# GoekeLab/m6anet

Hardware: AMD Instinct MI355X
Metric: DRACH sites/sec at num_iterations=1000 (higher is better)
Workload: dtype f32

## Files before the change

m6anet_amd/csrc/m6a_api.hip:

```cpp
#include "m6a_ctx.h"

#if !defined(__HIP_DEVICE_COMPILE__)
#ifndef M6A_MT_JUMP_PATH
#error "build with -DM6A_MT_JUMP_PATH=\"<repo>/m6anet_amd/assets/mt19937_jump.bin\" (m6anet_amd/build.py does)"
#endif
asm(".section .rodata\n"
    ".global m6a_mt_jump_blob\n.global m6a_mt_jump_blob_end\n.hidden m6a_mt_jump_blob\n.hidden m6a_mt_jump_blob_end\n.balign 64\n"
    "m6a_mt_jump_blob:\n.incbin \"" M6A_MT_JUMP_PATH "\"\n"
    "m6a_mt_jump_blob_end:\n.byte 0\n.previous\n");
#endif

namespace {

thread_local std::string g_create_error;

std::mutex g_live_mu;
std::vector<m6a_ctx *> g_live;
void join_background_setups()
{
    std::lock_guard<std::mutex> g(g_live_mu);
    for (m6a_ctx *c : g_live)
        if (c->warm.joinable()) c->warm.join();
    g_live.clear();
}
// ... 553 lines not shown
    hipLaunchKernelGGL(bag_verify_kernel, dim3(1), dim3(256), 0, st, c->d_minmax, c->d_hist, (unsigned long long)c->bag_min,
                       (unsigned long long)c->bag_max, (unsigned long long)c->n_reads, hash, c->d_err);
    HIPCHK(c, hipGetLastError());
    c->side_work = true;
    return M6A_OK;
}

int launch_encode(m6a_ctx *c, const float *X, const uint8_t *km, const int64_t *off, int64_t S,
                  int64_t R, float *rp)
{
    if (R <= 0 || S <= 0) return M6A_OK;
    EncArgs a;
    a.X = X; a.site_kmers = km; a.off = off; a.wfrag = c->d_wfrag; a.emb = c->d_emb; a.read_prob = rp;
    a.wfrag2 = c->d_wfrag2; a.w1e_tab = c->d_w1e; a.bn = c->d_w1e + M6A_W1E_FLOATS; a.err = c->d_err;
    a.n_sites = S; a.n_reads = R; a.n_tiles = (R + 31) / 32; a.b3 = c->b3;
    a.clk = c->prof.clk_for(0);
#ifdef M6A_AB_W3
    const int64_t max_waves = (int64_t)c->n_cu * 12;
#else
    const int64_t max_waves = (int64_t)c->n_cu * 8;
#endif
    a.tiles_per_wave = (a.n_tiles + max_waves - 1) / max_waves;
    const int64_t waves = (a.n_tiles + a.tiles_per_wave - 1) / a.tiles_per_wave;
    const unsigned blocks = (unsigned)((waves + 3) / 4);
    const bool fits32 = S < 0x7ffffff0LL && a.n_tiles < 0x7ffffff0LL;
    if (c->enc_variant == 2 && !fits32) return fail(c, M6A_EUNSUPPORTED, "12-slot encoder: more than 2^31 sites or tiles");
    const bool scalar_chain = c->bag_min >= M6A_CSITE_MIN_BAG && fits32;
    const bool csite = c->enc_variant == 2 || (c->enc_variant == 4 && scalar_chain);
    const bool site16 = !csite && c->enc_variant != 3 && scalar_chain;
    c->enc_variant_used = csite ? "csite12" : "general16";
// ... 831 lines not shown
```

m6anet_amd/csrc/m6a_ctx.h:

```cpp
#pragma once
#include <hip/hip_runtime.h>
#include <dlfcn.h>
#include <sys/mman.h>

#include <algorithm>
#include <atomic>
#include <cmath>
#include <cstdarg>
#include <cstdio>
#include <cstdlib>
#include <cstring>
#include <condition_variable>
#include <functional>
#include <memory>
#include <mutex>
#include <new>
#include <string>
#include <thread>
#include <vector>

#include "m6a.h"
#include "m6a_kernels.h"
#include "m6a_host_cpus.h"

// ... 193 lines not shown
    int rt_presize = 0;
    uint32_t rt_credit_seed = 0; int64_t rt_credit_A = 0, rt_credit = 0;
    struct Job {
        bool open = false;
        int failed = 0;
        std::string failed_msg;
        int T = 0, K = 0; float thr = 0.f; uint32_t seed = 0; int64_t bs = 1, spb = 1;
        std::vector<int64_t> off;
        int64_t S = 0, R = 0;
        int n_sub = 0; size_t sub_bytes = 0, o_goff = 0, o_km = 0, o_x = 0;
        int64_t cap_sites = 0, cap_reads = 0;
        std::vector<char *> pin;
        std::vector<hipEvent_t> ev_h2d, ev_enc;
        std::vector<char> used;
        int64_t item = 0;
        int64_t fill_sites = 0, fill_reads = 0, fill_min = INT64_MAX;
        bool cur_ready = false;
        int64_t chunks = 0;
    } job;
    DevBuf gSite, gMod, gP;
    DevBuf jX, jP, jOff;
    DevBuf mt_scratch; int64_t mt_polys_G = 0;
    std::vector<int> iter_of;
    std::thread warm;
    void *comm = nullptr;
    int comm_rank = 0, comm_world = 0;
    Profiler prof;
    const char *pool_variant = "none";
};

namespace m6a_detail {
// ... 44 lines not shown
```

m6anet_amd/csrc/m6a_job.hip:

```cpp
#include "m6a_ctx.h"

using namespace m6a_detail;

namespace m6a_detail {

int grow_keep(m6a_ctx *c, DevBuf &b, size_t used_bytes, size_t need_bytes)
{
    if (need_bytes <= b.cap) return M6A_OK;
    const size_t want = std::max(need_bytes + need_bytes / 8 + 256, b.cap * 2);
    void *np_ = nullptr;
    HIPCHK(c, hipMalloc(&np_, want));
    if (b.p && used_bytes) {
        if (c->stg.s_h2d) HIPCHK(c, hipStreamSynchronize(c->stg.s_h2d));
        HIPCHK(c, hipMemcpyAsync(np_, b.p, used_bytes, hipMemcpyDeviceToDevice, c->stream));
        HIPCHK(c, hipStreamSynchronize(c->stream));
    }
    if (b.p) (void)hipFree(b.p);
    b.p = np_; b.cap = want;
    return M6A_OK;
}

int job_setup_ring(m6a_ctx *c)
{
    auto &j = c->job;
// ... 52 lines not shown
    const int64_t ns = j.fill_sites, nr = j.fill_reads, s0 = j.S - ns, r0 = j.R - nr;
    int rc = grow_keep(c, c->jP, (size_t)r0 * 4, (size_t)std::max<int64_t>(j.R, 1) * 4);
    if (rc) return rc;
    rc = grow_keep(c, c->jOff, (size_t)(s0 + 1) * 8, (size_t)(j.S + 1) * 8);
    if (rc) return rc;
    if (j.used[(size_t)sub]) HIPCHK(c, hipStreamWaitEvent(g.s_h2d, j.ev_enc[(size_t)sub], 0));
    HIPCHK(c, hipMemcpyAsync(dev, pin, (size_t)(ns + 1) * 8, hipMemcpyHostToDevice, g.s_h2d));
    HIPCHK(c, hipMemcpyAsync((int64_t *)c->jOff.p + s0, pin + j.o_goff, (size_t)(ns + 1) * 8, hipMemcpyHostToDevice, g.s_h2d));
    if (!dX) {
        HIPCHK(c, hipMemcpyAsync(dev + j.o_km, pin + j.o_km, (size_t)ns * 3, hipMemcpyHostToDevice, g.s_h2d));
        if (nr) HIPCHK(c, hipMemcpyAsync(dev + j.o_x, pin + j.o_x, (size_t)nr * M6A_N_FEATURES * 4, hipMemcpyHostToDevice, g.s_h2d));
    }
    HIPCHK(c, hipEventRecord(j.ev_h2d[(size_t)sub], g.s_h2d));
    HIPCHK(c, hipStreamWaitEvent(c->stream, j.ev_h2d[(size_t)sub], 0));
    if (nr) {
        c->bag_min = j.fill_min; c->n_reads = nr;
        rc = launch_encode(c, dX ? dX : (const float *)(dev + j.o_x), dK ? dK : (const uint8_t *)(dev + j.o_km), (const int64_t *)dev, ns, nr,
                           (float *)c->jP.p + r0);
        if (rc) return rc;
    }
    HIPCHK(c, hipEventRecord(j.ev_enc[(size_t)sub], c->stream));
    j.used[(size_t)sub] = 1;
    j.item++; j.chunks++;
    j.fill_sites = 0; j.fill_reads = 0; j.fill_min = INT64_MAX; j.cur_ready = false;
    return M6A_OK;
}

void job_append_offsets(m6a_ctx *c, char *pin, const int64_t *off, int64_t i, int64_t k)
{
    auto &j = c->job;
    int64_t *ol = (int64_t *)pin, *og = (int64_t *)(pin + j.o_goff);
    if (j.fill_sites == 0) { ol[0] = 0; og[0] = j.R; }
    const int64_t base = off[i], lbase = j.fill_reads, gbase = j.R;
    int64_t mn = j.fill_min;
    for (int64_t t = 0; t < k; t++) {
        const int64_t e = off[i + t + 1] - base, n = off[i + t + 1] - off[i + t];
        ol[j.fill_sites + t + 1] = lbase + e;
        og[j.fill_sites + t + 1] = gbase + e;
        j.off.push_back(gbase + e);
        mn = n < mn ? n : mn;
    }
    j.fill_min = mn;
    const int64_t nr = off[i + k] - base;
    j.fill_sites += k; j.fill_reads += nr; j.S += k; j.R += nr;
}

int job_feed_impl(m6a_ctx *c, const float *X, const uint8_t *km, const int64_t *off, int64_t n, bool dev)
{
    auto &j = c->job;
    if (off[0] != 0) return fail(c, M6A_EINVAL, "off[0] must be 0");
    for (int64_t s = 0; s < n; s++) if (off[s + 1] < off[s]) return fail(c, M6A_EINVAL, "off[] must be non-decreasing");
    int rc;
    if (dev) {
        rc = job_flush(c);
        if (rc) return rc;
        for (int64_t i = 0; i < n;) {
            char *pin;
// ... 55 lines not shown
        return fail(c, M6A_EINVAL, "job offset %lld does not start a flush group for batch_size=%lld save_per_batch=%lld",
                    (long long)c->job_offset, (long long)bs, (long long)spb);
    HIPCHK(c, hipSetDevice(c->device));
    rc = job_setup_ring(c);
    if (rc) return rc;
    auto &j = c->job;
    j.T = T; j.K = K; j.thr = thr; j.seed = seed; j.bs = bs; j.spb = spb;
    try {
        j.off.clear();
        j.off.reserve((size_t)std::max<int64_t>(expect_sites, 1 << 16) + 1);
        j.off.push_back(0);
    } catch (const std::bad_alloc &) {
        return fail(c, M6A_ENOMEM, "out of host memory");
    }
    j.S = j.R = 0; j.item = 0; j.chunks = 0; j.failed = 0; j.failed_msg.clear();
    j.fill_sites = j.fill_reads = 0; j.fill_min = INT64_MAX; j.cur_ready = false;
    std::fill(j.used.begin(), j.used.end(), 0);
    HIPCHK(c, hipStreamSynchronize(c->stg.s_h2d));
    if (expect_reads) { rc = grow_keep(c, c->jP, 0, (size_t)expect_reads * 4); if (rc) return rc; }
    if (expect_sites) { rc = grow_keep(c, c->jOff, 0, (size_t)(expect_sites + 1) * 8); if (rc) return rc; }
    j.open = true;
    return M6A_OK;
}

int m6a_job_feed(m6a_ctx *c, const float *X, const uint8_t *km, const int64_t *off, int64_t n_sites)
{
    settle(c);
    if (!c) return M6A_EINVAL;
    auto &j = c->job;
    if (!j.open) return fail(c, M6A_EINVAL, "no streaming job is open (m6a_job_begin)");
    if (j.failed) { c->err = j.failed_msg; return j.failed; }
// ... 123 lines not shown
```

m6anet_amd/csrc/m6a_kernels.h:

```cpp
#ifndef M6A_KERNELS_H
#define M6A_KERNELS_H
#include <hip/hip_runtime.h>
#include <stdint.h>

#define M6A_BAG_LDS 1024
#define M6A_WFRAG_FLOATS (136 * 64)
#define M6A_WFRAG2_FLOATS (25 * 64)
#define M6A_W1E_FLOATS (35 * 32)
#define M6A_BN_FLOATS (5 * 2 * 16 * 2)
#define M6A_MEAN_STACK 32
#define M6A_CSITE_MIN_BAG 16
#define M6A_TABLE_MAX_N 32
#define M6A_REG_STACK 8
#define M6A_RTAB_MAX_N 4096
#define M6A_RTAB_SMALL_N 1024
#define M6A_RTAB_U8_MAX_N 256
#define M6A_HIST_BINS (M6A_RTAB_MAX_N + 2)

__host__ __device__ inline unsigned long long m6a_bin_weight(int i)
{
    unsigned long long z = (unsigned long long)(i + 1) * 0x9E3779B97F4A7C15ull;
    z = (z ^ (z >> 30)) * 0xBF58476D1CE4E5B9ull;
    z = (z ^ (z >> 27)) * 0x94D049BB133111EBull;
    return z ^ (z >> 31);
// ... 11 lines not shown
    }
}

struct EncArgs {
    const float *X;
    const uint8_t *site_kmers;
    const int64_t *off;
    const float *wfrag;
    const float *wfrag2;
    const float *w1e_tab;
    const float *bn;
    const float *emb;
    float *read_prob;
    int *err;
    int64_t n_sites, n_reads, n_tiles, tiles_per_wave;
    float b3;
    unsigned long long *clk;
};

struct PoolArgs {
    const float *read_prob;
    const int64_t *off;
    const int64_t *goff;
    const uint32_t *raw;
    const uint32_t *tab;
    float *site_prob;
    double *mod_ratio;
    uint32_t *start_pos;
    const int *leaf_start;
    const uint8_t *merge_after;
// ... 68 lines not shown
```

m6anet_amd/csrc/m6a_kernels.hip:

```cpp
#include <hip/hip_runtime.h>
#include <stdint.h>

#include "m6a_kernels.h"

typedef float f32x16 __attribute__((ext_vector_type(16)));
typedef float f32x2 __attribute__((ext_vector_type(2)));

__device__ __forceinline__ float chain8_sum(float r)
{
    r += __builtin_bit_cast(float, __builtin_amdgcn_update_dpp(0, __builtin_bit_cast(int, r), 0xB1, 0xf, 0xf, false));
    r += __builtin_bit_cast(float, __builtin_amdgcn_update_dpp(0, __builtin_bit_cast(int, r), 0x4E, 0xf, 0xf, false));
    r += __builtin_bit_cast(float, __builtin_amdgcn_update_dpp(0, __builtin_bit_cast(int, r), 0x141, 0xf, 0xf, false));
    return r;
}

__device__ __forceinline__ int wave_sum_i32(int v)
{
#pragma unroll
    for (int m = 1; m < 64; m <<= 1) v += __shfl_xor(v, m, 64);
    return v;
}

#define L2_REGS(m) ((m) == 4 ? 12 : 16)

// ... 50 lines not shown
__device__ __forceinline__ float bn_relu(float y, float alpha, float beta)
{
    float r;
    asm("v_fma_f32 %0, %1, %2, %3 clamp" : "=v"(r) : "v"(y), "v"(alpha), "v"(beta));
    return r;
}
#ifndef BN_BLOCK
#define BN_BLOCK 4
#endif
struct BnPairs { float4 v[BN_BLOCK / 2]; };
__device__ __forceinline__ void bn_pairs_load(BnPairs &pq, const float *p)
{
#pragma unroll
    for (int i = 0; i < BN_BLOCK / 2; i++) pq.v[i] = *(const float4 *)(p + 4 * i);
}
template <int M>
__device__ __forceinline__ void layer2_with_bn(f32x16 &acc2, f32x16 &cur, const float (&w2)[80], BnPairs &pq, const float *bn_half)
{
    constexpr int n = L2_REGS(M), m_next = M < 4 ? M + 1 : 0;
#pragma unroll
    for (int b = 0; b * BN_BLOCK < n; b++) {
#ifdef M6A_AB_PRIO_BLOCK_VALU
        __builtin_amdgcn_s_setprio(M6A_AB_PRIO_BLOCK_VALU);
#endif
#pragma unroll
        for (int i = 0; i < BN_BLOCK / 2; i++) {
            const int q = b * BN_BLOCK + 2 * i;
#ifdef M6A_AB_BN_PK
            f32x2 y = {cur[q], cur[q + 1]};
            const f32x2 al = {pq.v[i].x, pq.v[i].y}, be = {pq.v[i].z, pq.v[i].w};
            asm("v_pk_fma_f32 %0, %0, %1, %2 clamp" : "+v"(y) : "v"(al), "v"(be));
            cur[q] = y.x;
            cur[q + 1] = y.y;
#else
#ifndef M6A_AB_NO_BN
            cur[q] = bn_relu(cur[q], pq.v[i].x, pq.v[i].y);
            cur[q + 1] = bn_relu(cur[q + 1], pq.v[i].z, pq.v[i].w);
#endif
#endif
        }
#ifndef M6A_AB_NO_BN
        bn_pairs_load(pq, (b + 1) * BN_BLOCK < n ? bn_half + M * 64 + 2 * (b + 1) * BN_BLOCK : bn_half + m_next * 64);
#endif
        __builtin_amdgcn_sched_barrier(0);
#ifdef M6A_AB_PRIO_BLOCK_VALU
        __builtin_amdgcn_s_setprio(M6A_AB_PRIO_BLOCK_MFMA);
#endif
#pragma unroll
        for (int q = b * BN_BLOCK; q < (b + 1) * BN_BLOCK; q++)
            acc2 = __builtin_amdgcn_mfma_f32_32x32x2f32(w2[M * 16 + q], cur[q], acc2, 0, 0, 0);
        __builtin_amdgcn_sched_barrier(0);
    }
}

#ifdef M6A_AB_W3
template <int M>
__device__ __forceinline__ void layer2_with_bn_lds(f32x16 &acc2, f32x16 &cur, float4 (&wq)[2], const float4 *w2lane, BnPairs &pq, const float *bn_half)
{
    static_assert(BN_BLOCK == 4, "one float4 of A operands per block");
    constexpr int n = L2_REGS(M), m_next = M < 4 ? M + 1 : 0;
#pragma unroll
    for (int b = 0; b * 4 < n; b++) {
        const int g = M * 4 + b;
#pragma unroll
        for (int i = 0; i < 2; i++) {
// ... 60 lines not shown
#pragma unroll
    for (int q = 1; q < 7; q++) v[q] = r[8 + q] * w[8 + q];
    v[7] = half ? 0.0f : k0;
    c = ((v[0] + v[4]) + (v[2] + v[6])) + ((v[1] + v[5]) + (v[3] + v[7]));
    c_other = __shfl_xor(c, 32, 64);
    asm volatile("" : "+v"(c_other));
    return c + c_other;
}

__device__ __forceinline__ int64_t uniform_i64(int64_t v)
{
    return ((int64_t)__builtin_amdgcn_readfirstlane((int)(v >> 32)) << 32) |
           (uint32_t)__builtin_amdgcn_readfirstlane((int)v);
}

__device__ __forceinline__ void wave_lds_fence()
{
    __builtin_amdgcn_fence(__ATOMIC_ACQ_REL, "wavefront");
    __builtin_amdgcn_wave_barrier();
}

struct EncTile {
    float f[8];
    int64_t s_last;
};

__global__ __launch_bounds__(256, 2) void enc_kernel(EncArgs a)
{
    clamp_keeps_nan();
    m6a_clk_stamp(a.clk, 0);
// ... 4 lines not shown
    for (int i = threadIdx.x; i < M6A_BN_FLOATS; i += 256) s_bn[i] = a.bn[(i & ~3) | ((i & 1) << 1) | ((i & 2) >> 1)];
#else
    for (int i = threadIdx.x; i < M6A_BN_FLOATS; i += 256) s_bn[i] = a.bn[i];
#endif
    __syncthreads();

    const int lane = threadIdx.x & 63;
    const int col = lane & 31;
    const int half = lane >> 5;
    const float *bn_half = s_bn + half * 32;
    const int64_t wave = (int64_t)blockIdx.x * 4 + __builtin_amdgcn_readfirstlane((int)(threadIdx.x >> 6));
    const int64_t tile0 = wave * a.tiles_per_wave;
    if (tile0 >= a.n_tiles) return;
    const int64_t tile1 = (tile0 + a.tiles_per_wave < a.n_tiles) ? tile0 + a.tiles_per_wave : a.n_tiles;

    float w1[40], w2[80], w3[16];
#pragma unroll
    for (int i = 0; i < 40; i++) w1[i] = a.wfrag[i * 64 + lane];
#pragma unroll
    for (int i = 0; i < 80; i++) w2[i] = a.wfrag[(40 + i) * 64 + lane];
#pragma unroll
    for (int i = 0; i < 16; i++) w3[i] = a.wfrag[(120 + i) * 64 + lane];

    int64_t s_base;
    {
        const int64_t r = tile0 * 32;
        int64_t lo = 0, hi = a.n_sites;
        while (hi - lo > 1) {
            int64_t mid = (lo + hi) >> 1;
            if (a.off[mid] <= r) lo = mid; else hi = mid;
        }
        s_base = lo;
    }
    const int64_t last_site = a.n_sites - 1;

    auto link0 = [&](int64_t base, int64_t (&o)[3]) {
#pragma unroll
        for (int i = 0; i < 3; i++) {
            const int64_t si = base + 1 + i;
            o[i] = a.off[si <= a.n_sites ? si : a.n_sites];
        }
    };
    auto link1 = [&](int64_t tile, int64_t base, const int64_t (&o)[3], int64_t &s, int (&km)[3], float (&x)[8]) {
        const int64_t r = tile * 32 + col;
        const int64_t rc = r < a.n_reads ? r : a.n_reads - 1;
        s = base + (rc >= o[0] ? 1 : 0) + (rc >= o[1] ? 1 : 0);
        if (__any(rc >= o[2])) {
            s = base;
// ... 4 lines not shown
        km[0] = kp[0]; km[1] = kp[1]; km[2] = kp[2];
        const float *xp = a.X + rc * 9 + half;
#pragma unroll
        for (int i = 0; i < 4; i++) x[i] = xp[2 * i];
        x[4] = xp[half ? 6 : 8];
    };
    auto link2 = [&](const int (&km)[3], float (&x)[8]) {
        const float e0 = s_emb[2 * km[0] + 1 - half], e1 = s_emb[2 * km[1] + 1 - half], e2 = s_emb[2 * km[2] + 1 - half];
        x[4] = half ? e0 : x[4];
        x[5] = half ? e1 : e0;
        x[6] = half ? e2 : e1;
        x[7] = half ? 1.0f : e2;
    };

    float f[8];
    s_base = uniform_i64(s_base);
    {
        int64_t o[3], s;
        int km[3];
        link0(s_base, o);
        link1(tile0, s_base, o, s, km, f);
        link2(km, f);
        s_base = uniform_i64(__shfl(s, 31, 64));
    }

    BnPairs bnq;
    bn_pairs_load(bnq, bn_half);
    for (int64_t tile = tile0; tile < tile1; ++tile) {
        const int64_t tn = tile + 1 < tile1 ? tile + 1 : tile;
        float fn[8];
        int64_t o[3], sn;
        int km[3];
        link0(s_base, o);
        tile_body_priority();

        f32x16 acc2, h1a, h1b;
#pragma unroll
        for (int q = 0; q < 16; q++) { acc2[q] = 0.0f; h1a[q] = 0.0f; }
#pragma unroll
        for (int st = 0; st < 8; st++)
            h1a = __builtin_amdgcn_mfma_f32_32x32x2f32(w1[st], f[st], h1a, 0, 0, 0);
#pragma unroll
        for (int m = 0; m < 5; m++) {
            f32x16 &cur = (m & 1) ? h1b : h1a;
            f32x16 &nxt = (m & 1) ? h1a : h1b;
            if (m < 4) {
#pragma unroll
                for (int q = 0; q < 16; q++) nxt[q] = 0.0f;
#pragma unroll
                for (int st = 0; st < 8; st++)
                    nxt = __builtin_amdgcn_mfma_f32_32x32x2f32(w1[(m + 1) * 8 + st], f[st], nxt, 0, 0, 0);
            }
            __builtin_amdgcn_sched_barrier(0);
            if (m == 0) link1(tn, s_base, o, sn, km, fn);
            if (m == 2) link2(km, fn);
            if (m == 0) layer2_with_bn<0>(acc2, cur, w2, bnq, bn_half);
            if (m == 1) layer2_with_bn<1>(acc2, cur, w2, bnq, bn_half);
            if (m == 2) layer2_with_bn<2>(acc2, cur, w2, bnq, bn_half);
            if (m == 3) layer2_with_bn<3>(acc2, cur, w2, bnq, bn_half);
            if (m == 4) layer2_with_bn<4>(acc2, cur, w2, bnq, bn_half);
        }
        tile_epilogue_priority();
        const float z = gemv32_as_mkl(acc2, w3, half) + a.b3;
        const float p = 1.0f / (1.0f + sleef_expf_u10(-z));
        const int64_t r = tile * 32 + col;
        if (half == 0 && r < a.n_reads) a.read_prob[r] = p;
        if (tn != tile) s_base = uniform_i64(__shfl(sn, 31, 64));
#pragma unroll
        for (int i = 0; i < 8; i++) f[i] = fn[i];
    }
    m6a_clk_stamp(a.clk, 1);
}

#ifdef M6A_AB_STAMPS
#define M6A_AB_STAMP_TILES 16
// ... 32 lines not shown
#endif
    __syncthreads();

    const int lane = threadIdx.x & 63;
    const int col = lane & 31;
    const int half = lane >> 5;
    const float *bn_half = s_bn + half * 32;
    const int wave = (int)blockIdx.x * 4 + __builtin_amdgcn_readfirstlane((int)(threadIdx.x >> 6));
    const int n_tiles = (int)a.n_tiles, tpw = (int)a.tiles_per_wave;
    const int tile0 = wave * tpw;
    if (tile0 >= n_tiles) return;
    const int tile1 = (tile0 + tpw < n_tiles) ? tile0 + tpw : n_tiles;
    const int n_sites = (int)a.n_sites;
    const int last_lim = (int)(a.n_reads - 1 - (int64_t)(n_tiles - 1) * 32);

#ifdef M6A_AB_W3
    float w1[40], w3[16];
    float4 wq[2];
    const float4 *w2lane = s_w2q + lane;
    wq[0] = w2lane[0];
#pragma unroll
    for (int i = 0; i < 40; i++) w1[i] = a.wfrag[i * 64 + lane];
#else
    float w1[40], w2[80], w3[16];
#pragma unroll
    for (int i = 0; i < 40; i++) w1[i] = a.wfrag[i * 64 + lane];
#pragma unroll
    for (int i = 0; i < 80; i++) w2[i] = a.wfrag[(40 + i) * 64 + lane];
#endif
#pragma unroll
    for (int i = 0; i < 16; i++) w3[i] = a.wfrag[(120 + i) * 64 + lane];

    int s_base;
    {
        const int64_t r = (int64_t)tile0 * 32;
        int lo = 0, hi = n_sites;
        while (hi - lo > 1) {
            const int mid = (int)(((int64_t)lo + hi) >> 1);
            if (a.off[mid] <= r) lo = mid; else hi = mid;
        }
        s_base = lo;
    }
    const int last_site = n_sites - 1;

    const __attribute__((address_space(4))) int64_t *off_c = (const __attribute__((address_space(4))) int64_t *)a.off;
    auto link0 = [&](int base, int64_t (&o)[3]) {
#pragma unroll
        for (int i = 0; i < 3; i++) {
            const int si = base + 1 + i;
            o[i] = off_c[si <= n_sites ? si : n_sites];
        }
    };
    const int kq = lane < 18 ? lane : 17;
    const int kq_site = kq / 6, kq_byte = (kq % 6) / 2;
    int too_small = 0;
    auto link1 = [&](int tile, int base, const int64_t (&o)[3], int &rel, int &kid, float (&x)[8]) {
        const int64_t rbase = (int64_t)tile * 32;
// ... 24 lines not shown
    };
    auto link2 = [&](int kid, float &ev) { ev = s_emb[2 * kid + (lane & 1)]; };
    auto link3 = [&](float ev, int rel, float (&x)[8]) {
        const int ebits = __builtin_bit_cast(int, ev);
        const int addr = 4 * (rel * 6 + 1 - half);
        const float e0 = __builtin_bit_cast(float, __builtin_amdgcn_ds_bpermute(addr, ebits));
        const float e1 = __builtin_bit_cast(float, __builtin_amdgcn_ds_bpermute(addr + 8, ebits));
        const float e2 = __builtin_bit_cast(float, __builtin_amdgcn_ds_bpermute(addr + 16, ebits));
        x[4] = half ? e0 : x[4];
        x[5] = half ? e1 : e0;
        x[6] = half ? e2 : e1;
        x[7] = half ? 1.0f : e2;
    };

    float f[8];
    s_base = __builtin_amdgcn_readfirstlane(s_base);
    {
        int64_t o[3];
        int rel, kid;
        float ev;
        link0(s_base, o);
        link1(tile0, s_base, o, rel, kid, f);
        link2(kid, ev);
        link3(ev, rel, f);
        s_base += __builtin_amdgcn_readfirstlane(__shfl(rel, 31, 64));
    }

    phase_shift_second_workgroup();
    BnPairs bnq;
    bn_pairs_load(bnq, bn_half);
    for (int tile = tile0; tile < tile1; ++tile) {
        const int tn = tile + 1 < tile1 ? tile + 1 : tile;
        float fn[8], evn;
        int64_t o[3];
        int reln, kidn;
#ifdef M6A_AB_STAMPS
        unsigned long long ts[M6A_AB_STAMP_POINTS];
#endif
        M6A_STAMP(0);
        link0(s_base, o);
        tile_body_priority();

        f32x16 acc2, h1a, h1b;
#pragma unroll
        for (int q = 0; q < 16; q++) { acc2[q] = 0.0f; h1a[q] = 0.0f; }
#pragma unroll
        for (int st = 0; st < 8; st++)
            h1a = __builtin_amdgcn_mfma_f32_32x32x2f32(w1[st], f[st], h1a, 0, 0, 0);
        M6A_STAMP(1);
#pragma unroll
        for (int m = 0; m < 5; m++) {
            f32x16 &cur = (m & 1) ? h1b : h1a;
            f32x16 &nxt = (m & 1) ? h1a : h1b;
#ifndef M6A_AB_L2_FIRST
            if (m < 4) {
#pragma unroll
                for (int q = 0; q < 16; q++) nxt[q] = 0.0f;
#pragma unroll
                for (int st = 0; st < 8; st++)
                    nxt = __builtin_amdgcn_mfma_f32_32x32x2f32(w1[(m + 1) * 8 + st], f[st], nxt, 0, 0, 0);
            }
            __builtin_amdgcn_sched_barrier(0);
#endif
#ifndef M6A_AB_LINK1_AT
#define M6A_AB_LINK1_AT 1
#define M6A_AB_LINK2_AT 2
#define M6A_AB_LINK3_AT 3
#endif
#ifdef M6A_AB_NO_LINKS
            if (m == 0) {
#pragma unroll
                for (int i = 0; i < 8; i++) fn[i] = f[i];
                reln = 0; kidn = 0; evn = 0.0f;
            }
#else
            if (m == M6A_AB_LINK1_AT) link1(tn, s_base, o, reln, kidn, fn);
            if (m == M6A_AB_LINK2_AT) link2(kidn, evn);
            if (m == M6A_AB_LINK3_AT) link3(evn, reln, fn);
#endif
#ifdef M6A_AB_W3
            if (m == 0) layer2_with_bn_lds<0>(acc2, cur, wq, w2lane, bnq, bn_half);
            if (m == 1) layer2_with_bn_lds<1>(acc2, cur, wq, w2lane, bnq, bn_half);
            if (m == 2) layer2_with_bn_lds<2>(acc2, cur, wq, w2lane, bnq, bn_half);
            if (m == 3) layer2_with_bn_lds<3>(acc2, cur, wq, w2lane, bnq, bn_half);
            if (m == 4) layer2_with_bn_lds<4>(acc2, cur, wq, w2lane, bnq, bn_half);
#else
            if (m == 0) layer2_with_bn<0>(acc2, cur, w2, bnq, bn_half);
            if (m == 1) layer2_with_bn<1>(acc2, cur, w2, bnq, bn_half);
            if (m == 2) layer2_with_bn<2>(acc2, cur, w2, bnq, bn_half);
            if (m == 3) layer2_with_bn<3>(acc2, cur, w2, bnq, bn_half);
            if (m == 4) layer2_with_bn<4>(acc2, cur, w2, bnq, bn_half);
#endif
#ifdef M6A_AB_L2_FIRST
            if (m < 4) {
#pragma unroll
                for (int q = 0; q < 16; q++) nxt[q] = 0.0f;
#pragma unroll
                for (int st = 0; st < 8; st++)
                    nxt = __builtin_amdgcn_mfma_f32_32x32x2f32(w1[(m + 1) * 8 + st], f[st], nxt, 0, 0, 0);
            }
            __builtin_amdgcn_sched_barrier(0);
#endif
            M6A_STAMP(2 + m);
        }
        tile_epilogue_priority();
#ifdef M6A_AB_NO_EPILOGUE
        const float p = (acc2[0] + acc2[5]) + w3[0];
#else
        const float z = gemv32_as_mkl(acc2, w3, half) + a.b3;
        M6A_STAMP(7);
        const float p = 1.0f / (1.0f + sleef_expf_u10(-z));
#endif
        if (half == 0 && col <= (tile == n_tiles - 1 ? last_lim : 31)) (a.read_prob + (int64_t)tile * 32)[col] = p;
        M6A_STAMP(8);
// ... 37 lines not shown
    if (threadIdx.x < 64) s_w3[(threadIdx.x >> 5) * 16 + (threadIdx.x & 15)] = a.wfrag[(120 + (threadIdx.x & 15)) * 64 + (threadIdx.x & 32)];
    __syncthreads();

    const int lane = threadIdx.x & 63;
    const int col = lane & 31;
    const int half = lane >> 5;
    const float *bn_half = s_bn + half * 32;
    const int wave = (int)blockIdx.x * 4 + __builtin_amdgcn_readfirstlane((int)(threadIdx.x >> 6));
    const int n_tiles = (int)a.n_tiles, tpw = (int)a.tiles_per_wave;
    const int tile0 = wave * tpw;
    if (tile0 >= n_tiles) return;
    const int tile1 = (tile0 + tpw < n_tiles) ? tile0 + tpw : n_tiles;
    const int n_sites = (int)a.n_sites;
    const int last_lim = (int)(a.n_reads - 1 - (int64_t)(n_tiles - 1) * 32);

    float w1x[20], w8[5], w2[80];
#pragma unroll
    for (int i = 0; i < 20; i++) w1x[i] = a.wfrag2[i * 64 + lane];
#pragma unroll
    for (int i = 0; i < 5; i++) w8[i] = a.wfrag2[(20 + i) * 64 + lane];
#pragma unroll
    for (int i = 0; i < 80; i++) w2[i] = a.wfrag[(40 + i) * 64 + lane];

    int s_base;
    {
        const int64_t r = (int64_t)tile0 * 32;
        int lo = 0, hi = n_sites;
        while (hi - lo > 1) {
            const int mid = (int)(((int64_t)lo + hi) >> 1);
            if (a.off[mid] <= r) lo = mid; else hi = mid;
        }
        s_base = lo;
    }
    const int last_site = n_sites - 1;

    const __attribute__((address_space(4))) int64_t *off_c = (const __attribute__((address_space(4))) int64_t *)a.off;
    auto link0 = [&](int base, int64_t (&o)[3]) {
#pragma unroll
        for (int i = 0; i < 3; i++) {
            const int si = base + 1 + i;
            o[i] = off_c[si <= n_sites ? si : n_sites];
        }
    };
    const int kq = lane < 18 ? lane : 17;
    const int kq_site = kq / 6, kq_byte = (kq % 6) / 2;
    int too_small = 0;
    auto link1 = [&](int tile, int base, const int64_t (&o)[3], int &rel, int &kid, float (&x)[5]) {
        const int64_t rbase = (int64_t)tile * 32;
        const int lim = tile == n_tiles - 1 ? last_lim : 31;
// ... 60 lines not shown
            asm volatile("" : "+v"(a4[m]), "+v"(a5[m]));
#endif
        }
        x[4] = half ? (rel == 0 ? 1.0f : 0.0f) : x8;
        x[5] = (rel == (half ? 2 : 1)) ? 1.0f : 0.0f;
    };

    float f[6], a4[5], a5[5];
    s_base = __builtin_amdgcn_readfirstlane(s_base);
    {
        int64_t o[3];
        int rel, kid;
        float ev, x5[5];
        link0(s_base, o);
        link1(tile0, s_base, o, rel, kid, x5);
#pragma unroll
        for (int i = 0; i < 4; i++) f[i] = x5[i];
        link2(kid, ev);
        link3(ev, rel, x5[4], f, a4, a5);
        s_base += __builtin_amdgcn_readfirstlane(__shfl(rel, 31, 64));
    }

    BnPairs bnq;
    bn_pairs_load(bnq, bn_half);
    for (int tile = tile0; tile < tile1; ++tile) {
        const int tn = tile + 1 < tile1 ? tile + 1 : tile;
        float fn[5], evn;
        int64_t o[3];
        int reln, kidn;
        link0(s_base, o);
        tile_body_priority();

        auto layer1 = [&](int m, f32x16 &acc) {
#pragma unroll
            for (int q = 0; q < 16; q++) acc[q] = 0.0f;
#pragma unroll
            for (int st = 0; st < 4; st++)
                acc = __builtin_amdgcn_mfma_f32_32x32x2f32(w1x[m * 4 + st], f[st], acc, 0, 0, 0);
            acc = __builtin_amdgcn_mfma_f32_32x32x2f32(a4[m], f[4], acc, 0, 0, 0);
            acc = __builtin_amdgcn_mfma_f32_32x32x2f32(a5[m], f[5], acc, 0, 0, 0);
        };

        f32x16 acc2, h1a, h1b;
#pragma unroll
        for (int q = 0; q < 16; q++) acc2[q] = 0.0f;
        layer1(0, h1a);
#pragma unroll
        for (int m = 0; m < 5; m++) {
            f32x16 &cur = (m & 1) ? h1b : h1a;
            f32x16 &nxt = (m & 1) ? h1a : h1b;
            if (m < 4) layer1(m + 1, nxt);
            __builtin_amdgcn_sched_barrier(0);
            if (m == 0) link1(tn, s_base, o, reln, kidn, fn);
            if (m == 1) link2(kidn, evn);
            if (m == 3) link3(evn, reln, fn[4], f, a4, a5);
            if (m == 0) layer2_with_bn<0>(acc2, cur, w2, bnq, bn_half);
            if (m == 1) layer2_with_bn<1>(acc2, cur, w2, bnq, bn_half);
            if (m == 2) layer2_with_bn<2>(acc2, cur, w2, bnq, bn_half);
            if (m == 3) layer2_with_bn<3>(acc2, cur, w2, bnq, bn_half);
            if (m == 4) layer2_with_bn<4>(acc2, cur, w2, bnq, bn_half);
        }
        tile_epilogue_priority();
        float z = 0.0f;
#pragma unroll
        for (int q = 0; q < 16; q++) z = fmaf(relu2(acc2[q]), s_w3[half * 16 + q], z);
        z += __shfl_xor(z, 32, 64);
        z += a.b3;
        const float p = 1.0f / (1.0f + expf(-z));
        if (half == 0 && col <= (tile == n_tiles - 1 ? last_lim : 31)) (a.read_prob + (int64_t)tile * 32)[col] = p;
        if (tn != tile) s_base += __builtin_amdgcn_readfirstlane(__shfl(reln, 31, 64));
#pragma unroll
        for (int i = 0; i < 4; i++) f[i] = fn[i];
    }
    if (too_small && lane == 0) atomicExch(a.err, 2);
    m6a_clk_stamp(a.clk, 1);
// ... 662 lines not shown
```

Before: 387.5 million.

## Narrow first-site search with bag bounds and defer weight loads past prologue

Adds a bag-size-bounded range for the per-wave binary search of the first site, loading offsets via scalar constant loads. Weight fragment loads are moved after the first tile's offset and feature loads, so the dependent prologue chain is issued first, followed by a full wait before the tile loop. It also adds an optional (macro-gated) interleaving of layer-1 MFMA chains into the layer-2 MFMA stream. The woven-chain path is off by default; the explicit full waitcnt may add some stall.

Result: no change. 386.5 million (-0.3%).

```diff
diff --git a/m6anet_amd/csrc/m6a_api.hip b/m6anet_amd/csrc/m6a_api.hip
--- a/m6anet_amd/csrc/m6a_api.hip
+++ b/m6anet_amd/csrc/m6a_api.hip
@@ -591,6 +591,7 @@
     a.X = X; a.site_kmers = km; a.off = off; a.wfrag = c->d_wfrag; a.emb = c->d_emb; a.read_prob = rp;
     a.wfrag2 = c->d_wfrag2; a.w1e_tab = c->d_w1e; a.bn = c->d_w1e + M6A_W1E_FLOATS; a.err = c->d_err;
     a.n_sites = S; a.n_reads = R; a.n_tiles = (R + 31) / 32; a.b3 = c->b3;
+    a.bag_min = c->bag_min; a.bag_max = c->bag_max;
     a.clk = c->prof.clk_for(0);
 #ifdef M6A_AB_W3
     const int64_t max_waves = (int64_t)c->n_cu * 12;
diff --git a/m6anet_amd/csrc/m6a_ctx.h b/m6anet_amd/csrc/m6a_ctx.h
--- a/m6anet_amd/csrc/m6a_ctx.h
+++ b/m6anet_amd/csrc/m6a_ctx.h
@@ -231,7 +231,7 @@
         std::vector<hipEvent_t> ev_h2d, ev_enc;
         std::vector<char> used;
         int64_t item = 0;
-        int64_t fill_sites = 0, fill_reads = 0, fill_min = INT64_MAX;
+        int64_t fill_sites = 0, fill_reads = 0, fill_min = INT64_MAX, fill_max = 0;
         bool cur_ready = false;
         int64_t chunks = 0;
     } job;
diff --git a/m6anet_amd/csrc/m6a_job.hip b/m6anet_amd/csrc/m6a_job.hip
--- a/m6anet_amd/csrc/m6a_job.hip
+++ b/m6anet_amd/csrc/m6a_job.hip
@@ -90,7 +90,7 @@
     HIPCHK(c, hipEventRecord(j.ev_h2d[(size_t)sub], g.s_h2d));
     HIPCHK(c, hipStreamWaitEvent(c->stream, j.ev_h2d[(size_t)sub], 0));
     if (nr) {
-        c->bag_min = j.fill_min; c->n_reads = nr;
+        c->bag_min = j.fill_min; c->bag_max = j.fill_max; c->n_reads = nr;
         rc = launch_encode(c, dX ? dX : (const float *)(dev + j.o_x), dK ? dK : (const uint8_t *)(dev + j.o_km), (const int64_t *)dev, ns, nr,
                            (float *)c->jP.p + r0);
         if (rc) return rc;
@@ -98,7 +98,7 @@
     HIPCHK(c, hipEventRecord(j.ev_enc[(size_t)sub], c->stream));
     j.used[(size_t)sub] = 1;
     j.item++; j.chunks++;
-    j.fill_sites = 0; j.fill_reads = 0; j.fill_min = INT64_MAX; j.cur_ready = false;
+    j.fill_sites = 0; j.fill_reads = 0; j.fill_min = INT64_MAX; j.fill_max = 0; j.cur_ready = false;
     return M6A_OK;
 }
 
@@ -108,15 +108,16 @@
     int64_t *ol = (int64_t *)pin, *og = (int64_t *)(pin + j.o_goff);
     if (j.fill_sites == 0) { ol[0] = 0; og[0] = j.R; }
     const int64_t base = off[i], lbase = j.fill_reads, gbase = j.R;
-    int64_t mn = j.fill_min;
+    int64_t mn = j.fill_min, mx = j.fill_max;
     for (int64_t t = 0; t < k; t++) {
         const int64_t e = off[i + t + 1] - base, n = off[i + t + 1] - off[i + t];
         ol[j.fill_sites + t + 1] = lbase + e;
         og[j.fill_sites + t + 1] = gbase + e;
         j.off.push_back(gbase + e);
         mn = n < mn ? n : mn;
-    }
-    j.fill_min = mn;
+        mx = n > mx ? n : mx;
+    }
+    j.fill_min = mn; j.fill_max = mx;
     const int64_t nr = off[i + k] - base;
     j.fill_sites += k; j.fill_reads += nr; j.S += k; j.R += nr;
 }
@@ -202,7 +203,7 @@
         return fail(c, M6A_ENOMEM, "out of host memory");
     }
     j.S = j.R = 0; j.item = 0; j.chunks = 0; j.failed = 0; j.failed_msg.clear();
-    j.fill_sites = j.fill_reads = 0; j.fill_min = INT64_MAX; j.cur_ready = false;
+    j.fill_sites = j.fill_reads = 0; j.fill_min = INT64_MAX; j.fill_max = 0; j.cur_ready = false;
     std::fill(j.used.begin(), j.used.end(), 0);
     HIPCHK(c, hipStreamSynchronize(c->stg.s_h2d));
     if (expect_reads) { rc = grow_keep(c, c->jP, 0, (size_t)expect_reads * 4); if (rc) return rc; }
diff --git a/m6anet_amd/csrc/m6a_kernels.h b/m6anet_amd/csrc/m6a_kernels.h
--- a/m6anet_amd/csrc/m6a_kernels.h
+++ b/m6anet_amd/csrc/m6a_kernels.h
@@ -49,6 +49,7 @@
     float *read_prob;
     int *err;
     int64_t n_sites, n_reads, n_tiles, tiles_per_wave;
+    int64_t bag_min, bag_max;
     float b3;
     unsigned long long *clk;
 };
diff --git a/m6anet_amd/csrc/m6a_kernels.hip b/m6anet_amd/csrc/m6a_kernels.hip
--- a/m6anet_amd/csrc/m6a_kernels.hip
+++ b/m6anet_amd/csrc/m6a_kernels.hip
@@ -88,10 +88,19 @@
 #pragma unroll
     for (int i = 0; i < BN_BLOCK / 2; i++) pq.v[i] = *(const float4 *)(p + 4 * i);
 }
-template <int M>
-__device__ __forceinline__ void layer2_with_bn(f32x16 &acc2, f32x16 &cur, const float (&w2)[80], BnPairs &pq, const float *bn_half)
+#if !defined(M6A_AB_WOVEN_CHAINS) || defined(M6A_AB_L2_FIRST) || defined(M6A_AB_W3)
+#define M6A_SERIAL_CHAINS 1
+#endif
+__device__ constexpr int l1_slot(int k, int na) { return ((2 * k + 1) * BN_BLOCK / na + 1) / 2; }
+template <int M, int NL1, class L1>
+__device__ __forceinline__ void layer2_with_bn(f32x16 &acc2, f32x16 &cur, const float (&w2)[80], BnPairs &pq, const float *bn_half, L1 &&layer1_step)
 {
     constexpr int n = L2_REGS(M), m_next = M < 4 ? M + 1 : 0;
+#ifdef M6A_SERIAL_CHAINS
+    constexpr bool weave = false;
+#else
+    constexpr bool weave = M < 4;
+#endif
 #pragma unroll
     for (int b = 0; b * BN_BLOCK < n; b++) {
 #ifdef M6A_AB_PRIO_BLOCK_VALU
@@ -120,9 +129,18 @@
 #ifdef M6A_AB_PRIO_BLOCK_VALU
         __builtin_amdgcn_s_setprio(M6A_AB_PRIO_BLOCK_MFMA);
 #endif
-#pragma unroll
-        for (int q = b * BN_BLOCK; q < (b + 1) * BN_BLOCK; q++)
+        const int k0 = weave ? b * BN_BLOCK * NL1 / 16 : 0, k1 = weave ? (b + 1) * BN_BLOCK * NL1 / 16 : 0;
+#pragma unroll
+        for (int q = b * BN_BLOCK; q < (b + 1) * BN_BLOCK; q++) {
+#pragma unroll
+            for (int k = k0; k < k1; k++)
+                if (l1_slot(k - k0, k1 - k0) == q - b * BN_BLOCK) {
+                    layer1_step(k);
+                    __builtin_amdgcn_sched_barrier(0);
+                }
             acc2 = __builtin_amdgcn_mfma_f32_32x32x2f32(w2[M * 16 + q], cur[q], acc2, 0, 0, 0);
+            if (weave) __builtin_amdgcn_sched_barrier(0);
+        }
         __builtin_amdgcn_sched_barrier(0);
     }
 }
@@ -213,6 +231,32 @@
            (uint32_t)__builtin_amdgcn_readfirstlane((int)v);
 }
 
+__device__ __forceinline__ int64_t first_site(const int64_t *off, int64_t r, int64_t n_sites, int64_t bag_min, int64_t bag_max)
+{
+    const __attribute__((address_space(4))) int64_t *off_c = (const __attribute__((address_space(4))) int64_t *)off;
+    int64_t lo = 0, hi = n_sites;
+    if (bag_min > 0 && bag_max >= bag_min) {
+        const int64_t l = (int64_t)((uint64_t)r / (uint64_t)bag_max);
+        int64_t h = bag_min == bag_max ? l + 1 : (int64_t)((uint64_t)r / (uint64_t)bag_min) + 1;
+        h = h < n_sites ? h : n_sites;
+        if (l < h) {
+            int64_t ol = off_c[l], oh = off_c[h];
+            asm volatile("" : "+s"(ol), "+s"(oh));
+            if (ol <= r && r < oh) { lo = l; hi = h; }
+        }
+    }
+    while (hi - lo > 1) {
+        const int64_t mid = (lo + hi) >> 1;
+        if (off_c[mid] <= r) lo = mid; else hi = mid;
+    }
+    return lo;
+}
+
+__device__ __forceinline__ void prologue_loads_arrived()
+{
+    __builtin_amdgcn_s_waitcnt(0x0F70);
+}
+
 __device__ __forceinline__ void wave_lds_fence()
 {
     __builtin_amdgcn_fence(__ATOMIC_ACQ_REL, "wavefront");
@@ -247,24 +291,7 @@
     if (tile0 >= a.n_tiles) return;
     const int64_t tile1 = (tile0 + a.tiles_per_wave < a.n_tiles) ? tile0 + a.tiles_per_wave : a.n_tiles;
 
-    float w1[40], w2[80], w3[16];
-#pragma unroll
-    for (int i = 0; i < 40; i++) w1[i] = a.wfrag[i * 64 + lane];
-#pragma unroll
-    for (int i = 0; i < 80; i++) w2[i] = a.wfrag[(40 + i) * 64 + lane];
-#pragma unroll
-    for (int i = 0; i < 16; i++) w3[i] = a.wfrag[(120 + i) * 64 + lane];
-
-    int64_t s_base;
-    {
-        const int64_t r = tile0 * 32;
-        int64_t lo = 0, hi = a.n_sites;
-        while (hi - lo > 1) {
-            int64_t mid = (lo + hi) >> 1;
-            if (a.off[mid] <= r) lo = mid; else hi = mid;
-        }
-        s_base = lo;
-    }
+    int64_t s_base = first_site(a.off, tile0 * 32, a.n_sites, a.bag_min, a.bag_max);
     const int64_t last_site = a.n_sites - 1;
 
     auto link0 = [&](int64_t base, int64_t (&o)[3]) {
@@ -299,18 +326,28 @@
     };
 
     float f[8];
+    float w1[40], w2[80], w3[16];
     s_base = uniform_i64(s_base);
     {
         int64_t o[3], s;
         int km[3];
         link0(s_base, o);
         link1(tile0, s_base, o, s, km, f);
+        __builtin_amdgcn_sched_barrier(0);
+#pragma unroll
+        for (int i = 0; i < 40; i++) w1[i] = a.wfrag[i * 64 + lane];
+#pragma unroll
+        for (int i = 0; i < 80; i++) w2[i] = a.wfrag[(40 + i) * 64 + lane];
+#pragma unroll
+        for (int i = 0; i < 16; i++) w3[i] = a.wfrag[(120 + i) * 64 + lane];
+        __builtin_amdgcn_sched_barrier(0);
         link2(km, f);
         s_base = uniform_i64(__shfl(s, 31, 64));
     }
 
     BnPairs bnq;
     bn_pairs_load(bnq, bn_half);
+    prologue_loads_arrived();
     for (int64_t tile = tile0; tile < tile1; ++tile) {
         const int64_t tn = tile + 1 < tile1 ? tile + 1 : tile;
         float fn[8];
@@ -329,21 +366,23 @@
         for (int m = 0; m < 5; m++) {
             f32x16 &cur = (m & 1) ? h1b : h1a;
             f32x16 &nxt = (m & 1) ? h1a : h1b;
+            auto l1 = [&](int st) { nxt = __builtin_amdgcn_mfma_f32_32x32x2f32(w1[(m < 4 ? m + 1 : 0) * 8 + st], f[st], nxt, 0, 0, 0); };
             if (m < 4) {
 #pragma unroll
                 for (int q = 0; q < 16; q++) nxt[q] = 0.0f;
-#pragma unroll
-                for (int st = 0; st < 8; st++)
-                    nxt = __builtin_amdgcn_mfma_f32_32x32x2f32(w1[(m + 1) * 8 + st], f[st], nxt, 0, 0, 0);
+#ifdef M6A_SERIAL_CHAINS
+#pragma unroll
+                for (int st = 0; st < 8; st++) l1(st);
+#endif
             }
             __builtin_amdgcn_sched_barrier(0);
             if (m == 0) link1(tn, s_base, o, sn, km, fn);
             if (m == 2) link2(km, fn);
-            if (m == 0) layer2_with_bn<0>(acc2, cur, w2, bnq, bn_half);
-            if (m == 1) layer2_with_bn<1>(acc2, cur, w2, bnq, bn_half);
-            if (m == 2) layer2_with_bn<2>(acc2, cur, w2, bnq, bn_half);
-            if (m == 3) layer2_with_bn<3>(acc2, cur, w2, bnq, bn_half);
-            if (m == 4) layer2_with_bn<4>(acc2, cur, w2, bnq, bn_half);
+            if (m == 0) layer2_with_bn<0, 8>(acc2, cur, w2, bnq, bn_half, l1);
+            if (m == 1) layer2_with_bn<1, 8>(acc2, cur, w2, bnq, bn_half, l1);
+            if (m == 2) layer2_with_bn<2, 8>(acc2, cur, w2, bnq, bn_half, l1);
+            if (m == 3) layer2_with_bn<3, 8>(acc2, cur, w2, bnq, bn_half, l1);
+            if (m == 4) layer2_with_bn<4, 8>(acc2, cur, w2, bnq, bn_half, l1);
         }
         tile_epilogue_priority();
         const float z = gemv32_as_mkl(acc2, w3, half) + a.b3;
@@ -406,33 +445,7 @@
     const int n_sites = (int)a.n_sites;
     const int last_lim = (int)(a.n_reads - 1 - (int64_t)(n_tiles - 1) * 32);
 
-#ifdef M6A_AB_W3
-    float w1[40], w3[16];
-    float4 wq[2];
-    const float4 *w2lane = s_w2q + lane;
-    wq[0] = w2lane[0];
-#pragma unroll
-    for (int i = 0; i < 40; i++) w1[i] = a.wfrag[i * 64 + lane];
-#else
-    float w1[40], w2[80], w3[16];
-#pragma unroll
-    for (int i = 0; i < 40; i++) w1[i] = a.wfrag[i * 64 + lane];
-#pragma unroll
-    for (int i = 0; i < 80; i++) w2[i] = a.wfrag[(40 + i) * 64 + lane];
-#endif
-#pragma unroll
-    for (int i = 0; i < 16; i++) w3[i] = a.wfrag[(120 + i) * 64 + lane];
-
-    int s_base;
-    {
-        const int64_t r = (int64_t)tile0 * 32;
-        int lo = 0, hi = n_sites;
-        while (hi - lo > 1) {
-            const int mid = (int)(((int64_t)lo + hi) >> 1);
-            if (a.off[mid] <= r) lo = mid; else hi = mid;
-        }
-        s_base = lo;
-    }
+    int s_base = (int)first_site(a.off, (int64_t)tile0 * 32, a.n_sites, a.bag_min, a.bag_max);
     const int last_site = n_sites - 1;
 
     const __attribute__((address_space(4))) int64_t *off_c = (const __attribute__((address_space(4))) int64_t *)a.off;
@@ -487,6 +500,13 @@
     };
 
     float f[8];
+#ifdef M6A_AB_W3
+    float w1[40], w3[16];
+    float4 wq[2];
+    const float4 *w2lane = s_w2q + lane;
+#else
+    float w1[40], w2[80], w3[16];
+#endif
     s_base = __builtin_amdgcn_readfirstlane(s_base);
     {
         int64_t o[3];
@@ -494,6 +514,20 @@
         float ev;
         link0(s_base, o);
         link1(tile0, s_base, o, rel, kid, f);
+        __builtin_amdgcn_sched_barrier(0);
+#ifdef M6A_AB_W3
+        wq[0] = w2lane[0];
+#pragma unroll
+        for (int i = 0; i < 40; i++) w1[i] = a.wfrag[i * 64 + lane];
+#else
+#pragma unroll
+        for (int i = 0; i < 40; i++) w1[i] = a.wfrag[i * 64 + lane];
+#pragma unroll
+        for (int i = 0; i < 80; i++) w2[i] = a.wfrag[(40 + i) * 64 + lane];
+#endif
+#pragma unroll
+        for (int i = 0; i < 16; i++) w3[i] = a.wfrag[(120 + i) * 64 + lane];
+        __builtin_amdgcn_sched_barrier(0);
         link2(kid, ev);
         link3(ev, rel, f);
         s_base += __builtin_amdgcn_readfirstlane(__shfl(rel, 31, 64));
@@ -502,6 +536,7 @@
     phase_shift_second_workgroup();
     BnPairs bnq;
     bn_pairs_load(bnq, bn_half);
+    prologue_loads_arrived();
     for (int tile = tile0; tile < tile1; ++tile) {
         const int tn = tile + 1 < tile1 ? tile + 1 : tile;
         float fn[8], evn;
@@ -525,13 +560,15 @@
         for (int m = 0; m < 5; m++) {
             f32x16 &cur = (m & 1) ? h1b : h1a;
             f32x16 &nxt = (m & 1) ? h1a : h1b;
+            auto l1 = [&](int st) { nxt = __builtin_amdgcn_mfma_f32_32x32x2f32(w1[(m < 4 ? m + 1 : 0) * 8 + st], f[st], nxt, 0, 0, 0); };
 #ifndef M6A_AB_L2_FIRST
             if (m < 4) {
 #pragma unroll
                 for (int q = 0; q < 16; q++) nxt[q] = 0.0f;
-#pragma unroll
-                for (int st = 0; st < 8; st++)
-                    nxt = __builtin_amdgcn_mfma_f32_32x32x2f32(w1[(m + 1) * 8 + st], f[st], nxt, 0, 0, 0);
+#ifdef M6A_SERIAL_CHAINS
+#pragma unroll
+                for (int st = 0; st < 8; st++) l1(st);
+#endif
             }
             __builtin_amdgcn_sched_barrier(0);
 #endif
@@ -558,19 +595,18 @@
             if (m == 3) layer2_with_bn_lds<3>(acc2, cur, wq, w2lane, bnq, bn_half);
             if (m == 4) layer2_with_bn_lds<4>(acc2, cur, wq, w2lane, bnq, bn_half);
 #else
-            if (m == 0) layer2_with_bn<0>(acc2, cur, w2, bnq, bn_half);
-            if (m == 1) layer2_with_bn<1>(acc2, cur, w2, bnq, bn_half);
-            if (m == 2) layer2_with_bn<2>(acc2, cur, w2, bnq, bn_half);
-            if (m == 3) layer2_with_bn<3>(acc2, cur, w2, bnq, bn_half);
-            if (m == 4) layer2_with_bn<4>(acc2, cur, w2, bnq, bn_half);
+            if (m == 0) layer2_with_bn<0, 8>(acc2, cur, w2, bnq, bn_half, l1);
+            if (m == 1) layer2_with_bn<1, 8>(acc2, cur, w2, bnq, bn_half, l1);
+            if (m == 2) layer2_with_bn<2, 8>(acc2, cur, w2, bnq, bn_half, l1);
+            if (m == 3) layer2_with_bn<3, 8>(acc2, cur, w2, bnq, bn_half, l1);
+            if (m == 4) layer2_with_bn<4, 8>(acc2, cur, w2, bnq, bn_half, l1);
 #endif
 #ifdef M6A_AB_L2_FIRST
             if (m < 4) {
 #pragma unroll
                 for (int q = 0; q < 16; q++) nxt[q] = 0.0f;
 #pragma unroll
-                for (int st = 0; st < 8; st++)
-                    nxt = __builtin_amdgcn_mfma_f32_32x32x2f32(w1[(m + 1) * 8 + st], f[st], nxt, 0, 0, 0);
+                for (int st = 0; st < 8; st++) l1(st);
             }
             __builtin_amdgcn_sched_barrier(0);
 #endif
@@ -638,25 +674,9 @@
     const int n_sites = (int)a.n_sites;
     const int last_lim = (int)(a.n_reads - 1 - (int64_t)(n_tiles - 1) * 32);
 
+    int s_base = (int)first_site(a.off, (int64_t)tile0 * 32, a.n_sites, a.bag_min, a.bag_max);
+    const int last_site = n_sites - 1;
     float w1x[20], w8[5], w2[80];
-#pragma unroll
-    for (int i = 0; i < 20; i++) w1x[i] = a.wfrag2[i * 64 + lane];
-#pragma unroll
-    for (int i = 0; i < 5; i++) w8[i] = a.wfrag2[(20 + i) * 64 + lane];
-#pragma unroll
-    for (int i = 0; i < 80; i++) w2[i] = a.wfrag[(40 + i) * 64 + lane];
-
-    int s_base;
-    {
-        const int64_t r = (int64_t)tile0 * 32;
-        int lo = 0, hi = n_sites;
-        while (hi - lo > 1) {
-            const int mid = (int)(((int64_t)lo + hi) >> 1);
-            if (a.off[mid] <= r) lo = mid; else hi = mid;
-        }
-        s_base = lo;
-    }
-    const int last_site = n_sites - 1;
 
     const __attribute__((address_space(4))) int64_t *off_c = (const __attribute__((address_space(4))) int64_t *)a.off;
     auto link0 = [&](int base, int64_t (&o)[3]) {
@@ -747,6 +767,14 @@
         float ev, x5[5];
         link0(s_base, o);
         link1(tile0, s_base, o, rel, kid, x5);
+        __builtin_amdgcn_sched_barrier(0);
+#pragma unroll
+        for (int i = 0; i < 20; i++) w1x[i] = a.wfrag2[i * 64 + lane];
+#pragma unroll
+        for (int i = 0; i < 5; i++) w8[i] = a.wfrag2[(20 + i) * 64 + lane];
+#pragma unroll
+        for (int i = 0; i < 80; i++) w2[i] = a.wfrag[(40 + i) * 64 + lane];
+        __builtin_amdgcn_sched_barrier(0);
 #pragma unroll
         for (int i = 0; i < 4; i++) f[i] = x5[i];
         link2(kid, ev);
@@ -756,6 +784,7 @@
 
     BnPairs bnq;
     bn_pairs_load(bnq, bn_half);
+    prologue_loads_arrived();
     for (int tile = tile0; tile < tile1; ++tile) {
         const int tn = tile + 1 < tile1 ? tile + 1 : tile;
         float fn[5], evn;
@@ -764,34 +793,41 @@
         link0(s_base, o);
         tile_body_priority();
 
-        auto layer1 = [&](int m, f32x16 &acc) {
-#pragma unroll
-            for (int q = 0; q < 16; q++) acc[q] = 0.0f;
-#pragma unroll
-            for (int st = 0; st < 4; st++)
-                acc = __builtin_amdgcn_mfma_f32_32x32x2f32(w1x[m * 4 + st], f[st], acc, 0, 0, 0);
-            acc = __builtin_amdgcn_mfma_f32_32x32x2f32(a4[m], f[4], acc, 0, 0, 0);
-            acc = __builtin_amdgcn_mfma_f32_32x32x2f32(a5[m], f[5], acc, 0, 0, 0);
+        auto layer1_step = [&](int m, int st, f32x16 &acc) {
+            acc = __builtin_amdgcn_mfma_f32_32x32x2f32(st < 4 ? w1x[m * 4 + (st & 3)] : st == 4 ? a4[m] : a5[m], f[st], acc, 0, 0, 0);
         };
 
         f32x16 acc2, h1a, h1b;
 #pragma unroll
-        for (int q = 0; q < 16; q++) acc2[q] = 0.0f;
-        layer1(0, h1a);
+        for (int q = 0; q < 16; q++) { acc2[q] = 0.0f; h1a[q] = 0.0f; }
+#pragma unroll
+        for (int st = 0; st < 6; st++) layer1_step(0, st, h1a);
 #pragma unroll
         for (int m = 0; m < 5; m++) {
             f32x16 &cur = (m & 1) ? h1b : h1a;
             f32x16 &nxt = (m & 1) ? h1a : h1b;
-            if (m < 4) layer1(m + 1, nxt);
+            auto l1 = [&](int st) { layer1_step(m < 4 ? m + 1 : 0, st, nxt); };
+            if (m < 4) {
+#pragma unroll
+                for (int q = 0; q < 16; q++) nxt[q] = 0.0f;
+#ifdef M6A_SERIAL_CHAINS
+#pragma unroll
+                for (int st = 0; st < 6; st++) l1(st);
+#endif
+            }
             __builtin_amdgcn_sched_barrier(0);
             if (m == 0) link1(tn, s_base, o, reln, kidn, fn);
             if (m == 1) link2(kidn, evn);
+#ifdef M6A_SERIAL_CHAINS
             if (m == 3) link3(evn, reln, fn[4], f, a4, a5);
-            if (m == 0) layer2_with_bn<0>(acc2, cur, w2, bnq, bn_half);
-            if (m == 1) layer2_with_bn<1>(acc2, cur, w2, bnq, bn_half);
-            if (m == 2) layer2_with_bn<2>(acc2, cur, w2, bnq, bn_half);
-            if (m == 3) layer2_with_bn<3>(acc2, cur, w2, bnq, bn_half);
-            if (m == 4) layer2_with_bn<4>(acc2, cur, w2, bnq, bn_half);
+#else
+            if (m == 4) link3(evn, reln, fn[4], f, a4, a5);
+#endif
+            if (m == 0) layer2_with_bn<0, 6>(acc2, cur, w2, bnq, bn_half, l1);
+            if (m == 1) layer2_with_bn<1, 6>(acc2, cur, w2, bnq, bn_half, l1);
+            if (m == 2) layer2_with_bn<2, 6>(acc2, cur, w2, bnq, bn_half, l1);
+            if (m == 3) layer2_with_bn<3, 6>(acc2, cur, w2, bnq, bn_half, l1);
+            if (m == 4) layer2_with_bn<4, 6>(acc2, cur, w2, bnq, bn_half, l1);
         }
         tile_epilogue_priority();
         float z = 0.0f;
```
